# hungkq-1724/EraXviF5TTS

Hardware: AMD Instinct MI355X
Metric: mel-frames/s (higher is better)
Workload: dtype bf16; 1 GPU; C2 F5TTS_Base random-init, CFM.sample euler NFE=32 CFG=2 sway=-1, 32 utterances x seq_len 1024 (N_ref=341), one GPU, hipGraph=on; global_batch=32, per_gpu_batch=32, seq_len=1024, nfe=32, parallelism=utterance-sharded dp1, residual_stream=fp16 storage, fp32 arithmetic

## Files before the change

eraxvif5tts_amd/csrc/gemm_w4.hip:

```cpp
#include "gemm_tile.h"
#include "lnf_stats_math.h"
#include <string.h>

typedef _Float16 f16x4_t __attribute__((ext_vector_type(4)));

namespace {
constexpr int OPB = 32768;
constexpr int EPI_LDS_BYTES = 16384;

template <int EPI, bool LNF, int MI>
__global__ __launch_bounds__(256) __attribute__((amdgpu_waves_per_eu(1, 1))) void gemm_w4_kernel(GemmParams p, int tiles_n, int nblocks) {
    static_assert(EPI == EPI_STORE_T || EPI == EPI_ROPE_T || EPI == EPI_RESID, "block linears only");
    static_assert(!LNF || EPI != EPI_RESID, "LayerNorm fold: QKV (+ RoPE) and FF1 (+ GELU)");
    static_assert(MI == 8 || MI == 4, "token tiles per wave");
    constexpr int WROWS = MI * 16, BM = 2 * WROWS;
    constexpr int OPA = BM * 128;
    constexpr int WBASE = 2 * OPA, EPI_LDS = 2 * OPA + 2 * OPB;
    constexpr int NP = MI + 8, NR = MI + 8, NMF = 16 * MI;
    constexpr int LNF_AREA = MI == 4 ? 11264 : 2048;
    constexpr int EPI_BYTES = 4 * LNF_AREA > EPI_LDS_BYTES ? 4 * LNF_AREA : EPI_LDS_BYTES;
    __shared__ __attribute__((aligned(1024))) char smem[EPI_LDS + EPI_BYTES];
    const int tid = threadIdx.x, lane = tid & 63;
    const int wave = __builtin_amdgcn_readfirstlane(tid >> 6);
    const int wm = wave >> 1, wn = wave & 1;
    const int fr = lane & 15, fq = lane >> 4;

    auto tile_mn = [&](int bid, int& tm0, int& tn0) {
        const int q = nblocks >> 3, r = nblocks & 7, xcd = bid & 7;
        int swz = (xcd < r ? xcd * (q + 1) : r * (q + 1) + (xcd - r) * q) + (bid >> 3);
        if (p.tile_reverse) swz = nblocks - 1 - swz;
        const int gm = p.tile_group > 0 ? p.tile_group : 1;
        const int tiles_m_all = nblocks / tiles_n;
        const int grp = swz / (gm * tiles_n);
        const int gsz = min(gm, tiles_m_all - grp * gm);
        const int rin = swz - grp * gm * tiles_n;
        const int tile_n = rin / gsz, tile_m = grp * gm + (rin - tile_n * gsz);
        tm0 = tile_m * BM;
        tn0 = tile_n * 256;
    };
    [[maybe_unused]] unsigned pfv[4] = {0u, 0u, 0u, 0u};
    if constexpr (MI == 4) {
        if (p.pf_n[0] | p.pf_n[1]) {
#pragma unroll
            for (int r = 0; r < 2; ++r) {
                const size_t line = ((size_t)blockIdx.x * 2 + r) * 256u + tid;
                if (line * 128u < p.pf_n[0]) pfv[r] = *reinterpret_cast<const unsigned*>(static_cast<const char*>(p.pf_p[0]) + line * 128u);
                if (line * 128u < p.pf_n[1]) pfv[2 + r] = *reinterpret_cast<const unsigned*>(static_cast<const char*>(p.pf_p[1]) + line * 128u);
            }
        }
    }
    const int G = gridDim.x;
    const int my_tiles = (nblocks - (int)blockIdx.x + G - 1) / G;
    const int nk = p.K / 64;

    unsigned voffA[MI], voffW[8];
#pragma unroll
    for (int jj = 0; jj < 8; ++jj) {
        const int row = (wave * 8 + jj) * 8 + (lane >> 3);
        const int logical = (lane & 7) ^ ((row >> 1) & 7);
        voffW[jj] = (unsigned)(row * p.ldw * 2 + logical * 16);
    }
#pragma unroll
    for (int jj = 0; jj < MI; ++jj) {
        const int row = (wave * MI + jj) * 8 + (lane >> 3);
        const int logical = (lane & 7) ^ ((row >> 1) & 7);
        voffA[jj] = (unsigned)(row * p.lda * 2 + logical * 16);
    }
    const char* baseA;
    const char* baseW;
    int f_tile = blockIdx.x, f_k = 0;
    auto front_tile = [&]() {
        int sm, sn;
        tile_mn(f_tile, sm, sn);
        baseA = static_cast<const char*>(p.A) + (size_t)sm * p.lda * 2;
        baseW = static_cast<const char*>(p.W) + (size_t)sn * p.ldw * 2;
    };
    front_tile();
    const unsigned lds0 = (unsigned)(size_t)smem;
    const int wdstA = (int)lds0 + wave * MI * 1024, wdstW = (int)lds0 + WBASE + wave * 8192;
    auto dma16w = [&](int ldsdst, unsigned voff, const char* base) {
        asm volatile("s_mov_b32 m0, %0\n\ts_nop 0\n\tglobal_load_lds_dwordx4 %1, %2" ::"s"(ldsdst), "v"(voff), "s"(base) : "memory");
    };
    auto dma4w = [&](int ldsdst, unsigned voff, const void* base) {
        asm volatile("s_mov_b32 m0, %0\n\ts_nop 0\n\tglobal_load_lds_dword %1, %2" ::"s"(ldsdst), "v"(voff), "s"(base) : "memory");
    };
    auto front_advance = [&]() {
        baseA += 128;
        baseW += 128;
        if (++f_k == nk) {
            f_k = 0;
            f_tile += G;
            if (f_tile < nblocks) {
                front_tile();
            } else {
                f_tile -= G;
                baseA -= (size_t)nk * 128;
                baseW -= (size_t)nk * 128;
            }
        }
    };
    const unsigned ra0 = lds0 + (unsigned)((wm * WROWS + fr) * 128 + ((fq ^ (fr >> 1)) * 16));
    const unsigned ra1 = ra0 ^ 64u;
    const unsigned rw0 = lds0 + WBASE + (unsigned)((wn * 128 + fr) * 128 + ((fq ^ (fr >> 1)) * 16));
    const unsigned rw1 = rw0 ^ 64u;

    f32x4 acc[8][MI];
    f32x4 fw[2][8], fa[2][MI];
#define W4_DSR(dst, addr, off) asm volatile("ds_read_b128 %0, %1 offset:%2" : "=v"(dst) : "v"(addr), "n"(off))
    auto rd = [&](auto sc, auto xc, auto ec) {
        constexpr int S = decltype(sc)::value, X = decltype(xc)::value, e = decltype(ec)::value;
        (void)fw; (void)fa; (void)ra0; (void)ra1; (void)rw0; (void)rw1;
        if constexpr (e < 8) {
            if constexpr (S == 0) W4_DSR(fw[0][e], rw0, X * OPB + e * 2048); else W4_DSR(fw[1][e], rw1, X * OPB + e * 2048);
        } else {
            if constexpr (S == 0) W4_DSR(fa[0][e - 8], ra0, X * OPA + (e - 8) * 2048); else W4_DSR(fa[1][e - 8], ra1, X * OPA + (e - 8) * 2048);
        }
    };
    auto body = [&](auto xc, auto waitc) {
        constexpr int X = decltype(xc)::value;
        constexpr bool WAITV = decltype(waitc)::value;
        constexpr int R1S = 1, B1P = MI == 8 ? 20 : 13, D0 = MI == 8 ? 22 : 14, DS = MI == 8 ? 6 : 4, B2P = MI == 8 ? 86 : 42, R0 = MI == 8 ? 88 : 44,
                      R0S = MI == 8 ? 2 : 1;
        static_for<NMF>([&](auto nc) {
            (void)acc; (void)fw; (void)fa; (void)voffA; (void)voffW; (void)baseA; (void)baseW;
            constexpr int n = decltype(nc)::value;
            constexpr int s = n / (8 * MI), i = (n % (8 * MI)) / MI, j = n % MI;
            if constexpr (LNF)
                asm volatile("v_mfma_f32_16x16x32_f16 %0, %1, %2, %0" : "+a"(acc[i][j]) : "v"(fw[s][i]), "v"(fa[s][j]));
            else
                asm volatile("v_mfma_f32_16x16x32_bf16 %0, %1, %2, %0" : "+a"(acc[i][j]) : "v"(fw[s][i]), "v"(fa[s][j]));
            if constexpr (n < NR * R1S && n % R1S == 0) rd(std::integral_constant<int, 1>{}, xc, std::integral_constant<int, n / R1S>{});
            if constexpr (n == B1P) asm volatile("s_waitcnt lgkmcnt(0)\n\ts_barrier" ::: "memory");
            if constexpr (n >= D0 && n < D0 + NP * DS && (n - D0) % DS == 0) {
                constexpr int pc = (n - D0) / DS;
                if constexpr (pc < MI)
                    dma16w(X * OPA + wdstA + pc * 1024, voffA[pc], baseA);
                else
                    dma16w(X * OPB + wdstW + (pc - MI) * 1024, voffW[pc - MI], baseW);
            }
            if constexpr (n == B2P) {
                constexpr int issued = (B2P - D0) / DS + 1 > NP ? NP : (B2P - D0) / DS + 1;
                if constexpr (WAITV)
                    asm volatile("s_waitcnt vmcnt(%0)\n\ts_barrier" ::"n"(issued) : "memory");
                else
                    asm volatile("s_barrier" ::: "memory");
            }
            if constexpr (n >= R0 && n < R0 + NR * R0S && (n - R0) % R0S == 0)
                rd(std::integral_constant<int, 0>{}, std::integral_constant<int, 1 - X>{}, std::integral_constant<int, (n - R0) / R0S>{});
            if constexpr (n == NMF - 1) asm volatile("s_waitcnt lgkmcnt(0)" ::: "memory");
        });
        front_advance();
    };

    using T = std::true_type;
    using F = std::false_type;
    using X0 = std::integral_constant<int, 0>;
    using X1 = std::integral_constant<int, 1>;
    int m0, n0;
    tile_mn(blockIdx.x, m0, n0);
    char* const lnf_lds = smem + EPI_LDS + wave * LNF_AREA;
    [[maybe_unused]] auto stage_lnf = [&]() {
        const int ldst = (int)lds0 + EPI_LDS + wave * LNF_AREA;
        const unsigned nb = (unsigned)(n0 + wn * 128 + lane) * 4u;
        dma4w(ldst, nb, p.lnf_c1);
        dma4w(ldst + 256, nb + 256u, p.lnf_c1);
        dma4w(ldst + 512, nb, p.lnf_c2);
        dma4w(ldst + 768, nb + 256u, p.lnf_c2);
        if constexpr (MI == 4) {
            if (p.lnf_partial) {
                if (lane < 32) {
                    const unsigned ro = (unsigned)((m0 + wm * WROWS + 2 * lane) * 8);
#pragma unroll
                    for (int c = 0; c < 16; ++c)
                        dma16w(ldst + 2048 + c * 512, ro, reinterpret_cast<const char*>(p.lnf_partial + (size_t)c * p.lnf_partial_ld * 2));
                    if (p.lnf_pivot) dma16w(ldst + 2048 + 8192, ro, reinterpret_cast<const char*>(p.lnf_pivot));
                }
                return;
            }
        }
        dma16w(ldst + 1024, (unsigned)((m0 + wm * WROWS + 2 * lane) * 8), reinterpret_cast<const char*>(p.lnf_stats));
    };
    [[maybe_unused]] auto finish_stats = [&]() {
        if constexpr (MI == 4 && LNF) {
            if (p.lnf_partial) {
                float s1 = 0.f, s2 = 0.f;
#pragma unroll
                for (int c = 0; c < 16; ++c) {
                    const f32x2 v = *reinterpret_cast<const f32x2*>(lnf_lds + 2048 + c * 512 + lane * 8);
                    s1 += v[0];
                    s2 += v[1];
                }
                const float pv = p.lnf_pivot ? *reinterpret_cast<const float*>(lnf_lds + 2048 + 8192 + lane * 8) : 0.0f;
                float mean, rstd, sumsq;
                lnf_row_stats(s1, s2, pv, p.K, mean, rstd, sumsq);
                *reinterpret_cast<f32x2*>(lnf_lds + 1024 + lane * 8) = f32x2{mean, rstd};
                if (p.lnf_stats_out && n0 == 0 && wn == 0) {
                    const int m = m0 + wm * WROWS + lane;
                    const bool tok = p.lnf_rows == 0 || m + p.row0 < p.lnf_rows;
                    if (tok) *reinterpret_cast<f32x2*>(p.lnf_stats_out + (size_t)m * 2) = f32x2{mean, rstd};
                    lnf_raise_guard(p.lnf_sat, tok && !(sumsq < 65504.0f * 65504.0f), sumsq, p.lnf_sat_tag, m + p.row0);
                }
            }
        }
    };
    auto load_bias = [&](int tn0, f32x4 (&dst)[8]) {
#pragma unroll
        for (int i = 0; i < 8; ++i) dst[i] = *reinterpret_cast<const f32x4*>(p.bias + tn0 + wn * 128 + i * 16 + 4 * fq);
    };
    auto acc_from = [&](const f32x4 (&b4)[8]) {
        static_for<8>([&](auto ic) {
            static_for<MI>([&](auto jc) { acc[decltype(ic)::value][decltype(jc)::value] = b4[decltype(ic)::value]; });
        });
    };
#define W4_ACC(i, j)                                                                         \
    ([&]() -> f32x4 {                                                                        \
        float c0_, c1_, c2_, c3_;                                                            \
        asm volatile("v_accvgpr_read_b32 %0, %1" : "=v"(c0_) : "a"(acc[i][j][0]));           \
        asm volatile("v_accvgpr_read_b32 %0, %1" : "=v"(c1_) : "a"(acc[i][j][1]));           \
        asm volatile("v_accvgpr_read_b32 %0, %1" : "=v"(c2_) : "a"(acc[i][j][2]));           \
        asm volatile("v_accvgpr_read_b32 %0, %1" : "=v"(c3_) : "a"(acc[i][j][3]));           \
        return f32x4{c0_, c1_, c2_, c3_};                                                    \
    }())

    [[maybe_unused]] auto store_half_impl = [&](auto hc, auto actc, auto ropec) {
        constexpr int h = decltype(hc)::value, ACT = decltype(actc)::value;
        constexpr bool rope_wave = decltype(ropec)::value;
        const int nb = n0 + wn * 128 + h * 64;
        bf16_t* orow = reinterpret_cast<bf16_t*>(p.out_t) + (size_t)(m0 + wm * WROWS + fr) * p.ldo + nb + 16 * (fq & 1) + 8 * (fq >> 1);
        const size_t jstride = (size_t)16 * p.ldo;
        [[maybe_unused]] f32x4 rp[2][4];
        [[maybe_unused]] int pos0 = 0;
        auto load_rope = [&](auto jc, f32x4 (&dst)[4]) {
            constexpr int j = decltype(jc)::value;
            int pos = pos0 + 16 * j;
            pos -= pos >= p.rows_per_batch ? p.rows_per_batch : 0;
            const float* t = p.rope + (size_t)pos * 64 + 4 * fq;
#pragma unroll
            for (int i = 0; i < 4; ++i) dst[i] = *reinterpret_cast<const f32x4*>(t + 16 * i);
        };
        if constexpr (rope_wave) {
            pos0 = (p.row0 + m0 + wm * WROWS + fr) % p.rows_per_batch;
            load_rope(std::integral_constant<int, 0>{}, rp[0]);
        }
        [[maybe_unused]] f32x4 c1h[4], c2h[4];
        [[maybe_unused]] f32x2 stj[2];
        if constexpr (LNF) {
#pragma unroll
            for (int ii = 0; ii < 4; ++ii) {
                c1h[ii] = *reinterpret_cast<const f32x4*>(lnf_lds + ((h * 4 + ii) * 16 + 4 * fq) * 4);
                c2h[ii] = *reinterpret_cast<const f32x4*>(lnf_lds + 512 + ((h * 4 + ii) * 16 + 4 * fq) * 4);
            }
            stj[0] = *reinterpret_cast<const f32x2*>(lnf_lds + 1024 + fr * 8);
        }
        static_for<MI>([&](auto jc) {
            constexpr int j = decltype(jc)::value;
            __builtin_amdgcn_sched_barrier(0);
            if constexpr (LNF && j + 1 < MI) stj[(j + 1) & 1] = *reinterpret_cast<const f32x2*>(lnf_lds + 1024 + ((j + 1) * 16 + fr) * 8);
            if constexpr (rope_wave && j + 1 < MI) load_rope(std::integral_constant<int, j + 1>{}, rp[(j + 1) & 1]);
            f32x4 vals[4];
            static_for<4>([&](auto ic) {
                constexpr int ii = decltype(ic)::value, i = h * 4 + ii;
                f32x4 v = W4_ACC(i, j);
                if constexpr (LNF) v = epi_lnf4(v, stj[j & 1][0], stj[j & 1][1], c1h[ii], c2h[ii]);
                if constexpr (ACT == ACT_GELU_TANH) v = epi_gelu_tanh4(v);
                if constexpr (rope_wave) v = epi_rope4(v, rp[j & 1][ii]);
                vals[ii] = v;
            });
            const u32x4 q0 = pair_swap(to_bf16x4(vals[0]), to_bf16x4(vals[1]));
            const u32x4 q1 = pair_swap(to_bf16x4(vals[2]), to_bf16x4(vals[3]));
            bf16_t* o = orow + j * jstride;
            *reinterpret_cast<u32x4*>(o) = q0;
            *reinterpret_cast<u32x4*>(o + 32) = q1;
        });
    };
    [[maybe_unused]] auto store_half = [&](auto hc, auto actc) {
        if constexpr (EPI == EPI_ROPE_T) {
            const int nb = n0 + wn * 128 + decltype(hc)::value * 64;
            const int part = nb / p.rope_inner;
            if (part < 2 && ((nb - part * p.rope_inner) >> 6) < p.rope_heads) {
                store_half_impl(hc, actc, std::true_type{});
                return;
            }
        }
        store_half_impl(hc, actc, std::false_type{});
    };
    [[maybe_unused]] const float* const lds_bias = reinterpret_cast<const float*>(smem + EPI_LDS);
    [[maybe_unused]] const float* const lds_gate = lds_bias + p.N;
    [[maybe_unused]] auto emit_stats = [&](int nb, int m , float pivot, const f32x4& h0, const f32x4& h1, const f32x4& h2, const f32x4& h3) {
        const f32x4 npv{-pivot, -pivot, -pivot, -pivot};
        const f32x4 d0 = h0 + npv, d1 = h1 + npv, d2 = h2 + npv, d3 = h3 + npv;
        const f32x4 a = (d0 + d1) + (d2 + d3);
        const f32x4 q = __builtin_elementwise_fma(d3, d3, __builtin_elementwise_fma(d2, d2, __builtin_elementwise_fma(d1, d1, d0 * d0)));
        const float s1 = (a[0] + a[1]) + (a[2] + a[3]), s2 = (q[0] + q[1]) + (q[2] + q[3]);
        float a0 = s1, b0 = s2;
        asm volatile("s_nop 1\n\tv_permlane16_swap_b32 %0, %1" : "+v"(a0), "+v"(b0));
        float t = a0 + b0, z = 0.0f;
        asm volatile("s_nop 1\n\tv_permlane32_swap_b32 %0, %1" : "+v"(t), "+v"(z));
        const float tot = t + z;
        if (fq < 2) {
            char* sb = reinterpret_cast<char*>(p.stats_out + ((size_t)(nb >> 6) * p.stats_ld + (m0 + wm * WROWS)) * 2);
            *reinterpret_cast<float*>(sb + (unsigned)((m * 2 + fq) * 4)) = tot;
        }
    };
    [[maybe_unused]] auto resid_tile = [&]() {
        int fr = lane & 15, fq = lane >> 4;
        asm volatile("" : "+v"(fr), "+v"(fq));
        char* const sbase = reinterpret_cast<char*>(p.out_f) + ((size_t)(m0 + wm * WROWS) * p.ldof + n0 + wn * 128) * 2;
        unsigned offj[MI];
#pragma unroll
        for (int j = 0; j < MI; ++j) offj[j] = (unsigned)(((fr + 16 * j) * p.ldof + 16 * (fq & 1) + 8 * (fq >> 1)) * 2);
        unsigned keepbits = 0xffu;
        if (p.rowmask && p.rowbits) keepbits = ((unsigned)p.rowbits[((m0 + wm * WROWS) >> 7) * 16 + fr] >> (((m0 + wm * WROWS) & 127) >> 4)) & ((1u << MI) - 1u);
        float piv[MI];
        if (p.stats_out) {
            const float* pbase = p.stats_pivot ? p.stats_pivot + (size_t)(m0 + wm * WROWS) * 2 : nullptr;
#pragma unroll
            for (int j = 0; j < MI; ++j) piv[j] = pbase ? *reinterpret_cast<const float*>(reinterpret_cast<const char*>(pbase) + (unsigned)((fr + 16 * j) * 8)) : 0.0f;
        }
        u32x4 xs[2][MI][2];
        auto load_step = [&](auto sc) __attribute__((always_inline)) {
            constexpr int h = decltype(sc)::value / MI, j = decltype(sc)::value % MI;
            xs[h][j][0] = *reinterpret_cast<const u32x4*>(sbase + offj[j] + h * 128);
            xs[h][j][1] = *reinterpret_cast<const u32x4*>(sbase + offj[j] + h * 128 + 64);
        };
        constexpr int AHEAD = 4;
        static_for<AHEAD>([&](auto sc) { load_step(sc); });
        __builtin_amdgcn_sched_barrier(0);
        const bool all_kept = __builtin_amdgcn_ballot_w64(keepbits != ((1u << MI) - 1u)) == 0ull;
        auto widen_h = [](unsigned lo, unsigned hi) __attribute__((always_inline)) {
            const f16x4_t hv = __builtin_bit_cast(f16x4_t, u32x2{lo, hi});
            return f32x4{(float)hv[0], (float)hv[1], (float)hv[2], (float)hv[3]};
        };
        auto to_h16 = [](const f32x4& v) __attribute__((always_inline)) {
            f16x4_t hv;
#pragma unroll
            for (int e = 0; e < 4; ++e) hv[e] = (_Float16)__builtin_amdgcn_fmed3f(v[e], -65504.0f, 65504.0f);
            return hv;
        };
        auto h_f32 = [](const f16x4_t& hv) __attribute__((always_inline)) { return f32x4{(float)hv[0], (float)hv[1], (float)hv[2], (float)hv[3]}; };
        auto steps = [&](auto keptc) __attribute__((always_inline)) {
            constexpr bool ALL = decltype(keptc)::value;
            f32x4 g4[4];
            static_for<2 * MI>([&](auto sc) __attribute__((always_inline)) {
                constexpr int h = decltype(sc)::value / MI, j = decltype(sc)::value % MI;
                const int nb = n0 + wn * 128 + h * 64;
                if constexpr (j == 0) {
#pragma unroll
                    for (int ii = 0; ii < 4; ++ii) g4[ii] = *reinterpret_cast<const f32x4*>(lds_gate + nb + ii * 16 + 4 * fq);
                }
                f32x4 x0, x1, x2, x3;
                {
                    const u32x4 q = xs[h][j][0];
                    const u32x2 s0 = __builtin_amdgcn_permlane16_swap(q[0], q[2], false, false);
                    const u32x2 s1 = __builtin_amdgcn_permlane16_swap(q[1], q[3], false, false);
                    x0 = widen_h(s0[0], s1[0]);
                    x1 = widen_h(s0[1], s1[1]);
                }
                {
                    const u32x4 q = xs[h][j][1];
                    const u32x2 s0 = __builtin_amdgcn_permlane16_swap(q[0], q[2], false, false);
                    const u32x2 s1 = __builtin_amdgcn_permlane16_swap(q[1], q[3], false, false);
                    x2 = widen_h(s0[0], s1[0]);
                    x3 = widen_h(s0[1], s1[1]);
                }
                const f32x4 a0 = W4_ACC(h * 4 + 0, j), a1 = W4_ACC(h * 4 + 1, j), a2 = W4_ACC(h * 4 + 2, j), a3 = W4_ACC(h * 4 + 3, j);
                f32x4 v0 = epi_axpy4(a0, g4[0], x0), v1 = epi_axpy4(a1, g4[1], x1), v2 = epi_axpy4(a2, g4[2], x2), v3 = epi_axpy4(a3, g4[3], x3);
                if constexpr (!ALL) {
                    const bool keep = (keepbits >> j) & 1u;
                    v0 = keep ? v0 : x0;
                    v1 = keep ? v1 : x1;
                    v2 = keep ? v2 : x2;
                    v3 = keep ? v3 : x3;
                }
                const f16x4_t h0 = to_h16(v0), h1 = to_h16(v1), h2 = to_h16(v2), h3 = to_h16(v3);
                *reinterpret_cast<u32x4*>(sbase + offj[j] + h * 128) = pair_swap(__builtin_bit_cast(bf16x4, h0), __builtin_bit_cast(bf16x4, h1));
                *reinterpret_cast<u32x4*>(sbase + offj[j] + h * 128 + 64) = pair_swap(__builtin_bit_cast(bf16x4, h2), __builtin_bit_cast(bf16x4, h3));
                if (p.stats_out) emit_stats(nb, fr + 16 * j, piv[j], h_f32(h0), h_f32(h1), h_f32(h2), h_f32(h3));
                if constexpr (decltype(sc)::value + AHEAD < 2 * MI) load_step(std::integral_constant<int, decltype(sc)::value + AHEAD>{});
                __builtin_amdgcn_sched_barrier(0);
            });
        };
        if (all_kept)
            steps(std::true_type{});
        else
            steps(std::false_type{});
    };

    if constexpr (EPI == EPI_RESID) {
        float* lb = reinterpret_cast<float*>(smem + EPI_LDS);
        for (int i = tid; i < p.N; i += 256) {
            lb[i] = p.bias[i];
            lb[p.N + i] = p.gate ? p.gate[i] : 1.0f;
        }
    }
    auto issue_all = [&](int X) {
#pragma unroll
        for (int pc = 0; pc < MI; ++pc) dma16w(X * OPA + wdstA + pc * 1024, voffA[pc], baseA);
#pragma unroll
        for (int pc = 0; pc < 8; ++pc) dma16w(X * OPB + wdstW + pc * 1024, voffW[pc], baseW);
    };
    if constexpr (LNF) stage_lnf();
    issue_all(0);
    front_advance();
    issue_all(1);
    front_advance();
    f32x4 bstart[8];
    if constexpr (LNF) {
#pragma unroll
        for (int i = 0; i < 8; ++i) bstart[i] = f32x4{0.f, 0.f, 0.f, 0.f};
    } else {
        load_bias(n0, bstart);
    }
    acc_from(bstart);
    if constexpr (EPI == EPI_RESID) asm volatile("s_waitcnt lgkmcnt(0)" ::: "memory");
    asm volatile("s_waitcnt vmcnt(%0)\n\ts_barrier" ::"n"(NP) : "memory");
    static_for<NR>([&](auto ec) { rd(std::integral_constant<int, 0>{}, std::integral_constant<int, 0>{}, ec); });
    asm volatile("s_waitcnt lgkmcnt(0)" ::: "memory");

    for (int t = 0; t < my_tiles; ++t) {
        const bool last = t + 1 == my_tiles;
        if (t == 0)
            body(X0{}, T{});
        else
            body(X0{}, F{});
        body(X1{}, T{});
        for (int kt = 2; kt < nk; kt += 2) {
            body(X0{}, T{});
            body(X1{}, T{});
        }
        int nm0 = m0, nn0 = n0;
        if (!last) tile_mn(blockIdx.x + (t + 1) * G, nm0, nn0);
        if constexpr (EPI == EPI_RESID) {
            asm volatile("s_waitcnt vmcnt(0)" ::: "memory");
            __builtin_amdgcn_sched_barrier(0);
            resid_tile();
            __builtin_amdgcn_sched_barrier(0);
            f32x4 bn[8];
#pragma unroll
            for (int i = 0; i < 8; ++i) bn[i] = *reinterpret_cast<const f32x4*>(lds_bias + nn0 + wn * 128 + i * 16 + 4 * fq);
            acc_from(bn);
        } else {
            f32x4 bn[8];
            if constexpr (LNF) {
#pragma unroll
                for (int i = 0; i < 8; ++i) bn[i] = f32x4{0.f, 0.f, 0.f, 0.f};
            } else {
                load_bias(nn0, bn);
#pragma unroll
                for (int i = 0; i < 8; ++i) asm volatile("" ::"v"(bn[i]));
            }
            asm volatile("s_waitcnt vmcnt(0)" ::: "memory");
            __builtin_amdgcn_sched_barrier(0);
            finish_stats();
            if (p.act == ACT_GELU_TANH) {
                store_half(X0{}, std::integral_constant<int, ACT_GELU_TANH>{});
                store_half(X1{}, std::integral_constant<int, ACT_GELU_TANH>{});
            } else {
                store_half(X0{}, std::integral_constant<int, ACT_NONE>{});
                store_half(X1{}, std::integral_constant<int, ACT_NONE>{});
            }
            __builtin_amdgcn_sched_barrier(0);
            acc_from(bn);
        }
        m0 = nm0;
        n0 = nn0;
        if (!last) {
            static_for<NR>([&](auto ec) { rd(std::integral_constant<int, 0>{}, std::integral_constant<int, 0>{}, ec); });
            asm volatile("s_waitcnt lgkmcnt(0)" ::: "memory");
            if constexpr (LNF) stage_lnf();
        }
    }
    if constexpr (MI == 4) {
        if (((pfv[0] ^ pfv[1]) ^ (pfv[2] ^ pfv[3])) == 0x7fc0dead && (p.pf_n[0] | p.pf_n[1]) == 0xffffffffu) p.stats_out[0] = 0.f;
    }
#undef W4_ACC
#undef W4_DSR
}
}

int g_gemm_w4 = 1;
int g_gemm_w4_ink = 1;
int g_gemm_w4_bm = 0;

int gemm_persist_grid();

static int w4_tile_rows(const GemmParams& p) {
    const int pg = gemm_persist_grid();
    const int t256 = p.M % 256 == 0 ? (p.M / 256) * (p.N / 256) : 0, t128 = p.M % 128 == 0 ? (p.M / 128) * (p.N / 256) : 0;
    if (g_gemm_w4_bm == 256) return t256 >= pg ? 256 : 0;
    if (g_gemm_w4_bm == 128) return t128 >= pg ? 128 : 0;
    if (4 * t256 >= 3 * pg) return 256;
    return 2 * t128 >= pg ? 128 : 0;
}

int gemm_w4_lnf_inkernel(int M, int N, int K) {
    GemmParams t;
    memset(&t, 0, sizeof(t));
    t.M = M; t.N = N; t.K = K;
    if (!g_gemm_w4 || !g_gemm_w4_ink || K != 1024 || N % 256 != 0) return 0;
    const int rows = w4_tile_rows(t);
    if (rows == 128) return 128;
    return 0;
}

bool gemm_w4_ok(const GemmParams& p, int mode, int epi) {
    if (!g_gemm_w4 || mode != GEMM_DENSE) return false;
    if (p.N % 256 != 0 || p.K % 128 != 0 || p.K < 256 || (p.lda & 7) || (p.ldw & 7) || p.a_row_mod != 0 || p.row0 != 0) return false;
    if (w4_tile_rows(p) == 0) return false;
    if ((size_t)255 * (size_t)(p.lda > p.ldw ? p.lda : p.ldw) * 2 + 128 > 0x7fffffffull) return false;
    if (p.fin_counter) return false;
    if (p.lnf_partial && !(gemm_w4_lnf_inkernel(p.M, p.N, p.K) != 0 && p.lnf_stats && p.lnf_ncols == 16 && p.lnf_partial_ld >= p.M)) return false;
    const bool lnf = p.lnf_stats != nullptr;
    if (epi == EPI_STORE_T || epi == EPI_ROPE_T) {
        if (!p.out_t || (p.ldo & 7) || !(p.act == ACT_NONE || p.act == ACT_GELU_TANH)) return false;
        if (lnf ? (!p.lnf_c1 || !p.lnf_c2) : !p.bias) return false;
        if (epi == EPI_ROPE_T && (p.rows_per_batch < 128 || !p.rope || p.rope_inner % 64 != 0)) return false;
        return true;
    }
    if (epi == EPI_RESID) {
        if (lnf || !p.add2_f16 || !p.out_f || (p.ldof & 7) || p.act != ACT_NONE || !p.bias) return false;
        if ((p.gate && p.gate_bstride != 0) || (p.rowmask && !p.rowbits)) return false;
        if (p.stats_out && (p.N % 64 != 0 || p.stats_ld < p.M)) return false;
        if ((size_t)p.N * 8 > (size_t)EPI_LDS_BYTES) return false;
        return true;
    }
    return false;
}

template <int MI> static int launch_w4(const GemmParams& p, int epi, hipStream_t stream) {
    const int tiles_n = p.N / 256, nblocks = (p.M / (MI * 32)) * tiles_n;
    const int pg = gemm_persist_grid();
    const dim3 grid(nblocks < pg ? nblocks : pg), block(256);
    const bool lnf = p.lnf_stats != nullptr;
    if (epi == EPI_STORE_T && lnf)
        hipLaunchKernelGGL((gemm_w4_kernel<EPI_STORE_T, true, MI>), grid, block, 0, stream, p, tiles_n, nblocks);
    else if (epi == EPI_STORE_T)
        hipLaunchKernelGGL((gemm_w4_kernel<EPI_STORE_T, false, MI>), grid, block, 0, stream, p, tiles_n, nblocks);
    else if (epi == EPI_ROPE_T && lnf)
        hipLaunchKernelGGL((gemm_w4_kernel<EPI_ROPE_T, true, MI>), grid, block, 0, stream, p, tiles_n, nblocks);
    else if (epi == EPI_ROPE_T)
        hipLaunchKernelGGL((gemm_w4_kernel<EPI_ROPE_T, false, MI>), grid, block, 0, stream, p, tiles_n, nblocks);
    else if (epi == EPI_RESID)
        hipLaunchKernelGGL((gemm_w4_kernel<EPI_RESID, false, MI>), grid, block, 0, stream, p, tiles_n, nblocks);
    else
        return f5_fail(F5_EINVAL, "gemm_w4: unsupported epilogue %d", epi);
    F5_LAUNCH_CHECK();
    return 0;
}

int launch_gemm_w4(const GemmParams& p, int epi, hipStream_t stream) {
    return w4_tile_rows(p) == 128 ? launch_w4<4>(p, epi, stream) : launch_w4<8>(p, epi, stream);
}
```

eraxvif5tts_amd/csrc/ops.hip:

```cpp
#include <cstring>

#include "gemm.h"
#include "kernels.h"
#include "runtime.h"

static int sync_and_release(DevArena& a, hipStream_t st, int rc) {
    hipError_t e = hipStreamSynchronize(st);
    a.release();
    if (rc != 0) return rc;
    if (e != hipSuccess) return f5_fail(F5_EHIP, "stream synchronize failed: %s", hipGetErrorString(e));
    return 0;
}

extern "C" int f5_op_linear(int precision, int kernel, int M, int N, int K, const float* A, const float* W, const float* bias, int act,
                            float* out, f5_stream_t stream) {
    F5_TRY(f5_check_device());
    if (M <= 0 || N <= 0 || K <= 0 || !A || !W || !out) return f5_fail(F5_EINVAL, "bad argument");
    hipStream_t st = (hipStream_t)stream;
    const int Kp = (int)round_up(K, 64), Mp = (int)round_up(M, 256), Np = (int)round_up(N, 256);
    const size_t es = f5_elem_size(precision);
    DevArena a;
    void *At = nullptr, *Wt = nullptr;
    int rc = 0;
    do {
// ... 213 lines not shown
    if (precision != F5_PREC_BF16 && precision != F5_PREC_FP32) return f5_fail(F5_EINVAL, "bad precision %d", precision);
    if (ldx < dim || ldo < dim || (ldx & 3) || (ldo & 3) || (y && (ldy < dim || (ldy & 3)))) return f5_fail(F5_EINVAL, "leading dimensions below dim");
    if ((ymode != 0 && !y) || (ymode == 3 && !y2)) return f5_fail(F5_EINVAL, "residual mode %d needs its branches", ymode);
    if (inplace && xin_f16 != xout_f16) return f5_fail(F5_EINVAL, "in place needs one storage type");
    hipStream_t st = (hipStream_t)stream;
    const size_t es = f5_elem_size(precision), xn = (size_t)rows * ldx;
    DevArena a;
    void *xs = nullptr, *xo = nullptr, *ys = nullptr, *y2s = nullptr, *os = nullptr;
    unsigned* sat = nullptr;
    int rc = 0;
    do {
        if ((rc = a.alloc(&xs, xn * (xin_f16 ? 2 : 4)))) break;
        if ((rc = a.alloc(&os, (size_t)rows * ldo * es))) break;
        if ((rc = a.alloc_t(&sat, 8))) break;
        if (y && (rc = a.alloc(&ys, (size_t)rows * ldy * es))) break;
        if (y2 && (rc = a.alloc(&y2s, (size_t)rows * ldy * es))) break;
        if (inplace) xo = xs;
        else if ((rc = a.alloc(&xo, xn * (xout_f16 ? 2 : 4)))) break;
        if (xin_f16) {
            if ((rc = stage_f16(x, xs, xn, st))) break;
        } else {
            F5_HIP(hipMemcpyAsync(xs, x, xn * 4, hipMemcpyDeviceToDevice, st));
        }
        if (y && (rc = launch_convert_pad(precision, y, ldy, rows, ldy, ldy, ys, ldy, st))) break;
        if (y2 && (rc = launch_convert_pad(precision, y2, ldy, rows, ldy, ldy, y2s, ldy, st))) break;
        if ((rc = launch_layernorm_res(precision, xs, xin_f16, xo, xout_f16, ldx, rows, dim, ys, ldy, y2s, ymode, mul, add, mod_bstride, rows_per_batch,
                                       add_one, os, ldo, st, nullptr, guard ? sat : nullptr, sat_tag)))
            break;
        if ((rc = launch_convert_back(precision, os, ldo, rows, ldo, out, ldo, st))) break;
        if ((rc = xout_f16 ? launch_f16_to_f32(xo, xback, xn, st) : launch_convert_back(F5_PREC_FP32, xo, ldx, rows, ldx, xback, ldx, st))) break;
        if (guard) F5_HIP(hipMemcpyAsync(guard, sat, 6 * sizeof(unsigned), hipMemcpyDeviceToDevice, st));
    } while (0);
    return sync_and_release(a, st, rc);
}

extern "C" int f5_op_f32_to_f16(int64_t n, const float* src, float* dst, uint32_t* guard, f5_stream_t stream) {
    F5_TRY(f5_check_device());
    if (n <= 0 || !src || !dst) return f5_fail(F5_EINVAL, "bad argument");
    hipStream_t st = (hipStream_t)stream;
    DevArena a;
    void* h = nullptr;
    unsigned* sat = nullptr;
    int rc = 0;
    do {
        if ((rc = a.alloc(&h, (size_t)n * 2))) break;
        if ((rc = a.alloc_t(&sat, 8))) break;
        if ((rc = launch_f32_to_f16(src, h, (size_t)n, st, guard ? sat : nullptr))) break;
        if ((rc = launch_f16_to_f32(h, dst, (size_t)n, st))) break;
        if (guard) F5_HIP(hipMemcpyAsync(guard, sat, 6 * sizeof(unsigned), hipMemcpyDeviceToDevice, st));
    } while (0);
    return sync_and_release(a, st, rc);
}

extern "C" int f5_op_qknorm_rope(int precision, int rows, int heads, int rope_heads, int rows_per_batch, const float* qkv, const float* wq,
                                 const float* wk, const float* rope, float* out, f5_stream_t stream) {
    F5_TRY(f5_check_device());
    if (rows <= 0 || heads <= 0 || rope_heads < 0 || rope_heads > heads || rows_per_batch <= 0 || !qkv || !wq || !wk || !out || (rope_heads && !rope))
        return f5_fail(F5_EINVAL, "bad argument");
    if (precision != F5_PREC_BF16 && precision != F5_PREC_FP32) return f5_fail(F5_EINVAL, "bad precision %d", precision);
    hipStream_t st = (hipStream_t)stream;
    const int inner = heads * 64, ld = 3 * inner;
    DevArena a;
    void* q = nullptr;
    int rc = 0;
    do {
        if ((rc = a.alloc(&q, (size_t)rows * ld * f5_elem_size(precision)))) break;
        if ((rc = launch_convert_pad(precision, qkv, ld, rows, ld, ld, q, ld, st))) break;
        if ((rc = launch_qknorm_rope(precision, q, ld, rows, inner, heads, rope_heads, wq, wk, rope, rows_per_batch, st))) break;
        rc = launch_convert_back(precision, q, ld, rows, ld, out, ld, st);
    } while (0);
    return sync_and_release(a, st, rc);
}

extern "C" int f5_op_dwconv7_ln(int precision, int B, int N, int C, const float* x, const float* wt, const float* cbias, const float* ln_w,
                                const float* ln_b, float* out, f5_stream_t stream) {
    F5_TRY(f5_check_device());
    if (B <= 0 || N <= 0 || C <= 0 || !x || !wt || !cbias || !ln_w || !ln_b || !out) return f5_fail(F5_EINVAL, "bad argument");
    if (precision != F5_PREC_BF16 && precision != F5_PREC_FP32) return f5_fail(F5_EINVAL, "bad precision %d", precision);
    hipStream_t st = (hipStream_t)stream;
    const int rows = B * N;
    DevArena a;
    void* o = nullptr;
    int rc = 0;
    do {
        if ((rc = a.alloc(&o, (size_t)rows * C * f5_elem_size(precision)))) break;
        if ((rc = launch_dwconv7_ln(precision, x, B, N, C, wt, cbias, ln_w, ln_b, o, C, st))) break;
        rc = launch_convert_back(precision, o, C, rows, C, out, C, st);
    } while (0);
    return sync_and_release(a, st, rc);
}

extern "C" int f5_op_grn(int precision, int B, int N, int C, const float* h, const float* gamma, const float* beta, float* out, f5_stream_t stream) {
    F5_TRY(f5_check_device());
    if (B <= 0 || N <= 0 || C <= 0 || !h || !gamma || !beta || !out) return f5_fail(F5_EINVAL, "bad argument");
    if (precision != F5_PREC_BF16 && precision != F5_PREC_FP32) return f5_fail(F5_EINVAL, "bad precision %d", precision);
    hipStream_t st = (hipStream_t)stream;
    const int rows = B * N;
    DevArena a;
    void* hs = nullptr;
    float* scratch = nullptr;
    int rc = 0;
    do {
        if ((rc = a.alloc(&hs, (size_t)rows * C * f5_elem_size(precision)))) break;
        if ((rc = a.alloc_t(&scratch, (size_t)B * C + B))) break;
        if ((rc = launch_convert_pad(precision, h, C, rows, C, C, hs, C, st))) break;
        if ((rc = launch_grn(precision, hs, B, N, C, gamma, beta, scratch, st))) break;
        rc = launch_convert_back(precision, hs, C, rows, C, out, C, st);
    } while (0);
    return sync_and_release(a, st, rc);
}

extern "C" int f5_op_rmsnorm(int precision, int rows, int dim, const float* x, const float* g, float* out, f5_stream_t stream) {
    F5_TRY(f5_check_device());
    if (rows <= 0 || dim <= 0 || !x || !g || !out) return f5_fail(F5_EINVAL, "bad argument");
    if (precision != F5_PREC_BF16 && precision != F5_PREC_FP32) return f5_fail(F5_EINVAL, "bad precision %d", precision);
    hipStream_t st = (hipStream_t)stream;
    DevArena a;
    void* o = nullptr;
    int rc = 0;
    do {
        if ((rc = a.alloc(&o, (size_t)rows * dim * f5_elem_size(precision)))) break;
        if ((rc = launch_rmsnorm(precision, x, dim, rows, dim, g, o, dim, st))) break;
        rc = launch_convert_back(precision, o, dim, rows, dim, out, dim, st);
    } while (0);
    return sync_and_release(a, st, rc);
}

__global__ __launch_bounds__(256) void fill_random_kernel(uint16_t* dst, size_t n, uint32_t seed, float scale) {
    const size_t i = (size_t)blockIdx.x * 256 + threadIdx.x;
    if (i >= n) return;
    uint32_t x = (uint32_t)i * 2654435761u ^ seed;
    x ^= x >> 16; x *= 0x7feb352du; x ^= x >> 15; x *= 0x846ca68bu; x ^= x >> 16;
    const float u = ((float)(x >> 8) * (1.0f / 8388608.0f) - 1.0f) * scale;
    dst[i] = (uint16_t)(__float_as_uint(u) >> 16);
}
__global__ __launch_bounds__(256) void fill_random_f32_kernel(float* dst, size_t n, uint32_t seed, float scale) {
    const size_t i = (size_t)blockIdx.x * 256 + threadIdx.x;
    if (i >= n) return;
    uint32_t x = (uint32_t)i * 2654435761u ^ seed;
    x ^= x >> 16; x *= 0x7feb352du; x ^= x >> 15; x *= 0x846ca68bu; x ^= x >> 16;
    dst[i] = ((float)(x >> 8) * (1.0f / 8388608.0f) - 1.0f) * scale;
}

static int g_bench_pad_a = 0, g_bench_pad_w = 0;

extern "C" int f5_bench_gemm_site(int kernel, int site, int rows, int seq, int dim, int heads, int ff_inner, int iters, float* ms_avg,
                                  f5_stream_t stream) {
    F5_TRY(f5_check_device());
    if (!ms_avg || rows <= 0 || iters <= 0 || seq <= 0 || rows % seq != 0) return f5_fail(F5_EINVAL, "bad argument");
    hipStream_t st = (hipStream_t)stream;
    const int inner = heads * 64;
    int N, K, epi;
    switch (site) {
        case 0: N = 3 * inner; K = dim; epi = EPI_ROPE_T; break;
        case 1: N = ff_inner; K = dim; epi = EPI_STORE_T; break;
        case 2: N = dim; K = ff_inner; epi = EPI_GATE_T; break;
        case 3: N = dim; K = inner; epi = EPI_GATE_T; break;
        default: return f5_fail(F5_EINVAL, "bad site");
    }
    const size_t Mp = (size_t)round_up(rows, 256);
    const int lda = K + g_bench_pad_a, ldw = K + g_bench_pad_w;
    DevArena a;
    void *A = nullptr, *W = nullptr, *out = nullptr;
    float *bias = nullptr, *resid = nullptr, *gate = nullptr, *rope = nullptr;
    hipEvent_t e0 = nullptr, e1 = nullptr;
    int rc = 0;
    do {
        if ((rc = a.alloc(&A, Mp * lda * 2))) break;
        if ((rc = a.alloc(&W, (size_t)round_up(N, 256) * ldw * 2))) break;
        if ((rc = a.alloc(&out, Mp * N * 2))) break;
        if ((rc = a.alloc_t(&bias, (size_t)N))) break;
        if ((rc = a.alloc_t(&resid, Mp * (size_t)dim))) break;
        if ((rc = a.alloc_t(&gate, (size_t)dim))) break;
        if ((rc = a.alloc_t(&rope, (size_t)seq * 64))) break;
        hipLaunchKernelGGL(fill_random_kernel, dim3((unsigned)((Mp * lda + 255) / 256)), dim3(256), 0, st, (uint16_t*)A, Mp * lda, 1u, 1.0f);
        hipLaunchKernelGGL(fill_random_kernel, dim3((unsigned)(((size_t)N * ldw + 255) / 256)), dim3(256), 0, st, (uint16_t*)W, (size_t)N * ldw, 2u, 0.05f);
        hipLaunchKernelGGL(fill_random_f32_kernel, dim3((unsigned)((N + 255) / 256)), dim3(256), 0, st, bias, (size_t)N, 3u, 0.1f);
        hipLaunchKernelGGL(fill_random_f32_kernel, dim3((unsigned)((dim + 255) / 256)), dim3(256), 0, st, gate, (size_t)dim, 4u, 0.01f);
        hipLaunchKernelGGL(fill_random_f32_kernel, dim3((unsigned)((seq * 64 + 255) / 256)), dim3(256), 0, st, rope, (size_t)seq * 64, 5u, 0.7f);
        GemmParams g;
        memset(&g, 0, sizeof(g));
        g.A = A; g.lda = lda; g.W = W; g.ldw = ldw; g.M = rows; g.N = N; g.K = K; g.bias = bias; g.rows_per_batch = seq;
        g.site = N == 3 * K ? 1 : (N == K ? 2 : (N == 2 * K ? 3 : (K == 2 * N ? 4 : 0)));
        if (epi == EPI_ROPE_T) { g.out_t = out; g.ldo = N; g.rope = rope; g.rope_inner = inner; g.rope_heads = 1; }
        if (epi == EPI_STORE_T) { g.out_t = out; g.ldo = N; g.act = ACT_GELU_TANH; }
        if (epi == EPI_GATE_T) { g.out_t = out; g.ldo = N; g.gate = gate; g.gate_bstride = 0; }
        if (kernel == 1 && !gemm_fast_supported(g, F5_PREC_BF16, GEMM_DENSE, epi)) { rc = f5_fail(F5_ENOTSUP, "tuned kernel cannot run this site"); break; }
        if (hipEventCreate(&e0) != hipSuccess || hipEventCreate(&e1) != hipSuccess) { rc = f5_fail(F5_EHIP, "hipEventCreate failed"); break; }
        for (int i = 0; i < 2 && rc == 0; ++i) rc = launch_gemm(g, F5_PREC_BF16, GEMM_DENSE, epi, kernel, st);
        if (rc) break;
        (void)hipEventRecord(e0, st);
        for (int i = 0; i < iters && rc == 0; ++i) rc = launch_gemm(g, F5_PREC_BF16, GEMM_DENSE, epi, kernel, st);
        (void)hipEventRecord(e1, st);
        if (rc) break;
        if (hipEventSynchronize(e1) != hipSuccess) { rc = f5_fail(F5_EHIP, "event sync failed: %s", hipGetErrorString(hipGetLastError())); break; }
        float ms = 0.f;
        (void)hipEventElapsedTime(&ms, e0, e1);
        *ms_avg = ms / (float)iters;
    } while (0);
    if (e0) (void)hipEventDestroy(e0);
    if (e1) (void)hipEventDestroy(e1);
    return sync_and_release(a, st, rc);
}

extern "C" int f5_bench_attention(int kernel, int B, int N, int H, int iters, float* ms_avg, f5_stream_t stream) {
    F5_TRY(f5_check_device());
    if (!ms_avg || B <= 0 || N <= 0 || H <= 0 || iters <= 0) return f5_fail(F5_EINVAL, "bad argument");
    hipStream_t st = (hipStream_t)stream;
    const int inner = H * 64;
    const size_t rows = (size_t)B * N;
    DevArena a;
    void *q = nullptr, *o = nullptr;
    hipEvent_t e0 = nullptr, e1 = nullptr;
    int rc = 0;
    do {
        if ((rc = a.alloc(&q, rows * 3 * inner * 2))) break;
        if ((rc = a.alloc(&o, rows * inner * 2))) break;
        hipLaunchKernelGGL(fill_random_kernel, dim3((unsigned)((rows * 3 * inner + 255) / 256)), dim3(256), 0, st, (uint16_t*)q, rows * 3 * inner, 7u, 1.5f);
        if (kernel == 1 && !attention_fast_supported(F5_PREC_BF16, N, H)) { rc = f5_fail(F5_ENOTSUP, "tuned attention cannot run this shape"); break; }
        if (hipEventCreate(&e0) != hipSuccess || hipEventCreate(&e1) != hipSuccess) { rc = f5_fail(F5_EHIP, "hipEventCreate failed"); break; }
        for (int i = 0; i < 2 && rc == 0; ++i) rc = launch_attention(F5_PREC_BF16, kernel, B, N, H, q, 3 * inner, nullptr, o, inner, st);
        if (rc) break;
        (void)hipEventRecord(e0, st);
        for (int i = 0; i < iters && rc == 0; ++i) rc = launch_attention(F5_PREC_BF16, kernel, B, N, H, q, 3 * inner, nullptr, o, inner, st);
        (void)hipEventRecord(e1, st);
        if (rc) break;
        if (hipEventSynchronize(e1) != hipSuccess) { rc = f5_fail(F5_EHIP, "event sync failed"); break; }
        float ms = 0.f;
        (void)hipEventElapsedTime(&ms, e0, e1);
        *ms_avg = ms / (float)iters;
    } while (0);
    if (e0) (void)hipEventDestroy(e0);
    if (e1) (void)hipEventDestroy(e1);
    return sync_and_release(a, st, rc);
}

__global__ __launch_bounds__(256, 1) void mfma_rate_kernel(int iters, int random_operands, float* sink) {
    f32x4 acc[8][8];
#pragma unroll
    for (int i = 0; i < 8; ++i)
#pragma unroll
        for (int j = 0; j < 8; ++j) acc[i][j] = f32x4{0.f, 0.f, 0.f, 0.f};
    bf16x8 w[8], a[8];
    unsigned h = (threadIdx.x * 2654435761u) ^ (blockIdx.x * 40503u);
#pragma unroll
    for (int i = 0; i < 8; ++i)
#pragma unroll
        for (int e = 0; e < 8; ++e) {
            h = h * 1664525u + 1013904223u;
            w[i][e] = random_operands ? (bf16_t)(((int)(h >> 20) & 0xfff) * (1.0f / 1024.0f) - 2.0f) : (bf16_t)0.f;
            h = h * 1664525u + 1013904223u;
            a[i][e] = random_operands ? (bf16_t)(((int)(h >> 20) & 0xfff) * (1.0f / 32768.0f) - 0.0625f) : (bf16_t)0.f;
        }
    for (int it = 0; it < iters; ++it) {
#pragma unroll
        for (int i = 0; i < 8; ++i)
#pragma unroll
            for (int j = 0; j < 8; ++j)
                asm volatile("v_mfma_f32_16x16x32_bf16 %0, %1, %2, %0" : "+a"(acc[i][j]) : "v"(w[i]), "v"(a[j]));
    }
    asm volatile("s_nop 15\n\ts_nop 15" ::: "memory");
    float s = 0.f;
#pragma unroll
    for (int i = 0; i < 8; ++i)
#pragma unroll
        for (int j = 0; j < 8; ++j) s += acc[i][j][0];
    if (s == 12345.678f) sink[0] = s;
}

extern "C" int f5_bench_mfma_rate(int random_operands, float* tflops, f5_stream_t stream) {
    F5_TRY(f5_check_device());
    if (!tflops) return f5_fail(F5_EINVAL, "null argument");
    hipStream_t st = (hipStream_t)stream;
    int dev = 0, cus = 0;
    F5_HIP(hipGetDevice(&dev));
    F5_HIP(hipDeviceGetAttribute(&cus, hipDeviceAttributeMultiprocessorCount, dev));
    const int iters = 2000, blocks = cus * 4;
    DevArena a;
    float* sink = nullptr;
    hipEvent_t e0 = nullptr, e1 = nullptr;
    int rc = 0;
    do {
        if ((rc = a.alloc_t(&sink, 16))) break;
        if (hipEventCreate(&e0) != hipSuccess || hipEventCreate(&e1) != hipSuccess) { rc = f5_fail(F5_EHIP, "hipEventCreate failed"); break; }
        for (int i = 0; i < 3; ++i) hipLaunchKernelGGL(mfma_rate_kernel, dim3(blocks), dim3(256), 0, st, iters, random_operands, sink);
        (void)hipEventRecord(e0, st);
        const int reps = 10;
        for (int i = 0; i < reps; ++i) hipLaunchKernelGGL(mfma_rate_kernel, dim3(blocks), dim3(256), 0, st, iters, random_operands, sink);
        (void)hipEventRecord(e1, st);
        if (hipEventSynchronize(e1) != hipSuccess) { rc = f5_fail(F5_EHIP, "event sync failed"); break; }
        float ms = 0.f;
        (void)hipEventElapsedTime(&ms, e0, e1);
        const double flops = (double)reps * blocks * 4.0 * iters * 64.0 * (2.0 * 16 * 16 * 32);
        *tflops = (float)(flops / (ms * 1e-3) / 1e12);
    } while (0);
    if (e0) (void)hipEventDestroy(e0);
    if (e1) (void)hipEventDestroy(e1);
    return sync_and_release(a, st, rc);
}

extern int g_sync_evals, g_attn_persist, g_attn_stagger, g_resid_rmw, g_ln_fold, g_ln_fold_inkernel, g_ln_fold_fin, g_gemm_pad_rows;
extern int g_conv31_tok;
extern int g_gemm_bm128, g_gemm_tile, g_gemm_group_sites, g_gemm_reverse_sites;
extern int g_gemm_split_tail, g_gemm_w4, g_gemm_w4_bm, g_gemm_w4_ink;
extern int g_gemm_variant, g_gemm_group, g_gemm_persist_grid, g_gemm_persist, g_gemm_lean, g_ln_defer, g_ln_wide, g_ln_rows, g_ln_rows_min, g_w_prefetch, g_res_f16, g_conv31, g_attn_variant, g_vocos_fft;
int g_tuning_epoch = 0;
extern unsigned long long* g_attn_stamp_buf;
extern unsigned long long* g_gemm_clk_buf;
extern "C" int f5_debug_gemm_clock(void* dev_buf) {
    g_gemm_clk_buf = reinterpret_cast<unsigned long long*>(dev_buf);
    return 0;
}
extern "C" int f5_debug_attn_stamps(void* dev_buf) {
    g_attn_stamp_buf = reinterpret_cast<unsigned long long*>(dev_buf);
    return 0;
}

extern "C" int f5_tuning_set(const char* key, int value) {
    if (!key) return f5_fail(F5_EINVAL, "null key");
    ++g_tuning_epoch;
    if (strcmp(key, "gemm_variant") == 0) {
        g_gemm_variant = value;
        return 0;
    }
    if (strcmp(key, "resid_rmw") == 0) {
        g_resid_rmw = value != 0;
        return 0;
    }
    if (strcmp(key, "attn_stagger") == 0) {
        g_attn_stagger = value;
        return 0;
    }
    if (strcmp(key, "attn_persist") == 0) {
        g_attn_persist = value != 0;
        return 0;
    }
    if (strcmp(key, "sync_evals") == 0) {
        g_sync_evals = value != 0;
        return 0;
    }
    if (strcmp(key, "w_prefetch") == 0) {
        g_w_prefetch = value;
        return 0;
    }
    if (strcmp(key, "gemm_reverse_sites") == 0) {
        g_gemm_reverse_sites = value;
        return 0;
    }
    if (strcmp(key, "gemm_group_sites") == 0) {
        g_gemm_group_sites = value;
        return 0;
    }
    if (strcmp(key, "conv31_tok") == 0) {
        g_conv31_tok = value;
        return 0;
    }
    if (strcmp(key, "gemm_tile") == 0) {
        g_gemm_tile = value;
        return 0;
    }
    if (strcmp(key, "gemm_bm128") == 0) {
        g_gemm_bm128 = value;
        return 0;
    }
    if (strcmp(key, "ln_rows") == 0) {
        g_ln_rows = value;
        return 0;
    }
    if (strcmp(key, "ln_rows_min") == 0) {
        g_ln_rows_min = value;
        return 0;
    }
    if (strcmp(key, "ln_wide") == 0) {
        g_ln_wide = value != 0;
        return 0;
    }
    if (strcmp(key, "residual_f16") == 0) {
        g_res_f16 = value != 0;
        return 0;
    }
    if (strcmp(key, "vocos_fft") == 0) {
        g_vocos_fft = value != 0;
        return 0;
    }
    if (strcmp(key, "attn_variant") == 0) {
        g_attn_variant = value;
        return 0;
    }
    if (strcmp(key, "gemm_group") == 0) {
        g_gemm_group = value;
        return 0;
    }
    if (strcmp(key, "op_conv_kernel") == 0) {
        g_op_conv_kernel = value != 0;
        return 0;
    }
    if (strcmp(key, "conv31") == 0) {
        g_conv31 = value != 0;
        return 0;
    }
    if (strcmp(key, "ln_defer") == 0) {
        g_ln_defer = value != 0;
        return 0;
    }
    if (strcmp(key, "gemm_lean") == 0) {
        g_gemm_lean = value != 0;
        return 0;
    }
    if (strcmp(key, "gemm_pad_rows") == 0) {
        g_gemm_pad_rows = value != 0;
        return 0;
    }
    if (strcmp(key, "ln_fold_inkernel") == 0) {
        g_ln_fold_inkernel = value != 0;
        return 0;
    }
    if (strcmp(key, "ln_fold_fin") == 0) {
        g_ln_fold_fin = value != 0;
        return 0;
    }
    if (strcmp(key, "ln_fold") == 0) {
        g_ln_fold = value != 0;
        return 0;
    }
    if (strcmp(key, "gemm_split_tail") == 0) {
        g_gemm_split_tail = value != 0;
        return 0;
    }
    if (strcmp(key, "gemm_w4_ink") == 0) {
        g_gemm_w4_ink = value;
        return 0;
    }
    if (strcmp(key, "gemm_w4_bm") == 0) {
        g_gemm_w4_bm = value;
        return 0;
    }
    if (strcmp(key, "gemm_w4") == 0) {
        g_gemm_w4 = value != 0;
        return 0;
    }
    if (strcmp(key, "gemm_persist") == 0) {
        g_gemm_persist = value != 0;
        return 0;
    }
    if (strcmp(key, "gemm_persist_grid") == 0) {
        if (value != 0 && (value < 8 || value > 4096)) return f5_fail(F5_EINVAL, "gemm_persist_grid must be 0 (= CU count) or in [8, 4096]");
        g_gemm_persist_grid = value;
        return 0;
    }
    if (strcmp(key, "bench_pad_a") == 0) {
        g_bench_pad_a = value;
        return 0;
    }
    if (strcmp(key, "bench_pad_w") == 0) {
        g_bench_pad_w = value;
        return 0;
    }
    return f5_fail(F5_EINVAL, "unknown tuning key '%s'", key);
}
```

Before: 34090 mel-frames/s.

## Defer part of w4 GEMM epilogue stores into next tile's MFMA mainloop

In the persistent w4 GEMM with 256-row tiles, half of the odd token-tile epilogue results (16 u32x4 per wave) are now held in registers. They are written out with global_store_dwordx4 interleaved into the first K-iterations of the next tile, instead of being stored at once in the epilogue. The goal is to overlap epilogue store traffic with MFMA compute. The vmcnt waits are adjusted to count the drained stores, and any leftovers are flushed after the loop. It is enabled by default for RoPE QKV GEMMs only, and it adds register pressure and extra outstanding-store accounting.

```diff
diff --git a/eraxvif5tts_amd/csrc/gemm_w4.hip b/eraxvif5tts_amd/csrc/gemm_w4.hip
--- a/eraxvif5tts_amd/csrc/gemm_w4.hip
+++ b/eraxvif5tts_amd/csrc/gemm_w4.hip
@@ -6,13 +6,16 @@
 
 namespace {
 constexpr int OPB = 32768;
+constexpr int W4_DRAIN = 16;
 constexpr int EPI_LDS_BYTES = 16384;
 
-template <int EPI, bool LNF, int MI>
+template <int EPI, bool LNF, int MI, int ND = 0>
 __global__ __launch_bounds__(256) __attribute__((amdgpu_waves_per_eu(1, 1))) void gemm_w4_kernel(GemmParams p, int tiles_n, int nblocks) {
     static_assert(EPI == EPI_STORE_T || EPI == EPI_ROPE_T || EPI == EPI_RESID, "block linears only");
     static_assert(!LNF || EPI != EPI_RESID, "LayerNorm fold: QKV (+ RoPE) and FF1 (+ GELU)");
     static_assert(MI == 8 || MI == 4, "token tiles per wave");
+    static_assert(ND == 0 || (MI == 8 && EPI != EPI_RESID && ND % 4 == 0 && ND <= 16), "the drain: store-only epilogues of the 256-row tile");
+    constexpr int NJ = ND / 4, NDI = ND / 2;
     constexpr int WROWS = MI * 16, BM = 2 * WROWS;
     constexpr int OPA = BM * 128;
     constexpr int WBASE = 2 * OPA, EPI_LDS = 2 * OPA + 2 * OPB;
@@ -116,9 +119,17 @@
             if constexpr (S == 0) W4_DSR(fa[0][e - 8], ra0, X * OPA + (e - 8) * 2048); else W4_DSR(fa[1][e - 8], ra1, X * OPA + (e - 8) * 2048);
         }
     };
-    auto body = [&](auto xc, auto waitc) {
-        constexpr int X = decltype(xc)::value;
+    u32x4 dq[ND > 0 ? ND : 1];
+    [[maybe_unused]] const char* dbase = static_cast<const char*>(p.out_t);
+    [[maybe_unused]] unsigned doff[NJ > 0 ? NJ : 1];
+    if constexpr (ND > 0) {
+#pragma unroll
+        for (int e = 0; e < ND; ++e) dq[e] = u32x4{0u, 0u, 0u, 0u};
+    }
+    auto body = [&](auto xc, auto waitc, auto stc) {
+        constexpr int X = decltype(xc)::value, ST = decltype(stc)::value;
         constexpr bool WAITV = decltype(waitc)::value;
+        constexpr int DS0 = 97, DS1 = 109;
         constexpr int R1S = 1, B1P = MI == 8 ? 20 : 13, D0 = MI == 8 ? 22 : 14, DS = MI == 8 ? 6 : 4, B2P = MI == 8 ? 86 : 42, R0 = MI == 8 ? 88 : 44,
                       R0S = MI == 8 ? 2 : 1;
         static_for<NMF>([&](auto nc) {
@@ -140,13 +151,19 @@
             }
             if constexpr (n == B2P) {
                 constexpr int issued = (B2P - D0) / DS + 1 > NP ? NP : (B2P - D0) / DS + 1;
+                constexpr int drained = (ND > 0 && ST >= 0) ? (DS0 < B2P ? 1 : 0) + (DS1 < B2P ? 1 : 0) : 0;
                 if constexpr (WAITV)
-                    asm volatile("s_waitcnt vmcnt(%0)\n\ts_barrier" ::"n"(issued) : "memory");
+                    asm volatile("s_waitcnt vmcnt(%0)\n\ts_barrier" ::"n"(issued + drained) : "memory");
                 else
                     asm volatile("s_barrier" ::: "memory");
             }
             if constexpr (n >= R0 && n < R0 + NR * R0S && (n - R0) % R0S == 0)
                 rd(std::integral_constant<int, 0>{}, std::integral_constant<int, 1 - X>{}, std::integral_constant<int, (n - R0) / R0S>{});
+            if constexpr (ND > 0 && ST >= 0 && (n == DS0 || n == DS1)) {
+                constexpr int e = 2 * ST + (n == DS0 ? 0 : 1);
+                (void)dq; (void)doff; (void)dbase;
+                asm volatile("global_store_dwordx4 %0, %1, %2 offset:%3" ::"v"(doff[e / 4]), "v"(dq[e]), "s"(dbase), "n"(64 * (e % 4)) : "memory");
+            }
             if constexpr (n == NMF - 1) asm volatile("s_waitcnt lgkmcnt(0)" ::: "memory");
         });
         front_advance();
@@ -156,6 +173,7 @@
     using F = std::false_type;
     using X0 = std::integral_constant<int, 0>;
     using X1 = std::integral_constant<int, 1>;
+    using N1 = std::integral_constant<int, -1>;
     int m0, n0;
     tile_mn(blockIdx.x, m0, n0);
     char* const lnf_lds = smem + EPI_LDS + wave * LNF_AREA;
@@ -268,9 +286,14 @@
             });
             const u32x4 q0 = pair_swap(to_bf16x4(vals[0]), to_bf16x4(vals[1]));
             const u32x4 q1 = pair_swap(to_bf16x4(vals[2]), to_bf16x4(vals[3]));
-            bf16_t* o = orow + j * jstride;
-            *reinterpret_cast<u32x4*>(o) = q0;
-            *reinterpret_cast<u32x4*>(o + 32) = q1;
+            if constexpr (ND > 0 && (j & 1) && j / 2 < NJ) {
+                dq[(j / 2) * 4 + h * 2] = q0;
+                dq[(j / 2) * 4 + h * 2 + 1] = q1;
+            } else {
+                bf16_t* o = orow + j * jstride;
+                *reinterpret_cast<u32x4*>(o) = q0;
+                *reinterpret_cast<u32x4*>(o + 32) = q1;
+            }
         });
     };
     [[maybe_unused]] auto store_half = [&](auto hc, auto actc) {
@@ -419,14 +442,32 @@
 
     for (int t = 0; t < my_tiles; ++t) {
         const bool last = t + 1 == my_tiles;
-        if (t == 0)
-            body(X0{}, T{});
-        else
-            body(X0{}, F{});
-        body(X1{}, T{});
-        for (int kt = 2; kt < nk; kt += 2) {
-            body(X0{}, T{});
-            body(X1{}, T{});
+        if constexpr (ND == 0) {
+            if (t == 0)
+                body(X0{}, T{}, N1{});
+            else
+                body(X0{}, F{}, N1{});
+            body(X1{}, T{}, N1{});
+            for (int kt = 2; kt < nk; kt += 2) {
+                body(X0{}, T{}, N1{});
+                body(X1{}, T{}, N1{});
+            }
+        } else {
+            int kt = 0;
+            if (t > 0) {
+                static_for<NDI>([&](auto ic) {
+                    constexpr int it = decltype(ic)::value;
+                    if constexpr (it == 0)
+                        body(X0{}, F{}, ic);
+                    else
+                        body(std::integral_constant<int, it & 1>{}, T{}, ic);
+                });
+                kt = NDI;
+            }
+            for (; kt < nk; kt += 2) {
+                body(X0{}, T{}, N1{});
+                body(X1{}, T{}, N1{});
+            }
         }
         int nm0 = m0, nn0 = n0;
         if (!last) tile_mn(blockIdx.x + (t + 1) * G, nm0, nn0);
@@ -459,6 +500,11 @@
                 store_half(X0{}, std::integral_constant<int, ACT_NONE>{});
                 store_half(X1{}, std::integral_constant<int, ACT_NONE>{});
             }
+            if constexpr (ND > 0) {
+                dbase = static_cast<const char*>(p.out_t) + ((size_t)(m0 + wm * WROWS) * p.ldo + n0 + wn * 128) * 2;
+#pragma unroll
+                for (int jd = 0; jd < NJ; ++jd) doff[jd] = (unsigned)(((fr + 16 * (2 * jd + 1)) * p.ldo + 16 * (fq & 1) + 8 * (fq >> 1)) * 2);
+            }
             __builtin_amdgcn_sched_barrier(0);
             acc_from(bn);
         }
@@ -470,6 +516,12 @@
             if constexpr (LNF) stage_lnf();
         }
     }
+    if constexpr (ND > 0) {
+        static_for<ND>([&](auto ec) {
+            constexpr int e = decltype(ec)::value;
+            *reinterpret_cast<u32x4*>(const_cast<char*>(dbase) + doff[e / 4] + 64 * (e % 4)) = dq[e];
+        });
+    }
     if constexpr (MI == 4) {
         if (((pfv[0] ^ pfv[1]) ^ (pfv[2] ^ pfv[3])) == 0x7fc0dead && (p.pf_n[0] | p.pf_n[1]) == 0xffffffffu) p.stats_out[0] = 0.f;
     }
@@ -480,6 +532,7 @@
 
 int g_gemm_w4 = 1;
 int g_gemm_w4_ink = 1;
+int g_gemm_w4_drain = 1;
 int g_gemm_w4_bm = 0;
 
 int gemm_persist_grid();
@@ -532,6 +585,20 @@
     const int pg = gemm_persist_grid();
     const dim3 grid(nblocks < pg ? nblocks : pg), block(256);
     const bool lnf = p.lnf_stats != nullptr;
+    if constexpr (MI == 8) {
+        if ((epi == EPI_ROPE_T ? g_gemm_w4_drain >= 1 : epi == EPI_STORE_T && g_gemm_w4_drain >= 2) && nblocks > (int)grid.x && p.K >= 512 && (size_t)128 * (size_t)p.ldo * 2 < 0x7fffffffull) {
+            if (epi == EPI_STORE_T && lnf)
+                hipLaunchKernelGGL((gemm_w4_kernel<EPI_STORE_T, true, 8, W4_DRAIN>), grid, block, 0, stream, p, tiles_n, nblocks);
+            else if (epi == EPI_STORE_T)
+                hipLaunchKernelGGL((gemm_w4_kernel<EPI_STORE_T, false, 8, W4_DRAIN>), grid, block, 0, stream, p, tiles_n, nblocks);
+            else if (lnf)
+                hipLaunchKernelGGL((gemm_w4_kernel<EPI_ROPE_T, true, 8, W4_DRAIN>), grid, block, 0, stream, p, tiles_n, nblocks);
+            else
+                hipLaunchKernelGGL((gemm_w4_kernel<EPI_ROPE_T, false, 8, W4_DRAIN>), grid, block, 0, stream, p, tiles_n, nblocks);
+            F5_LAUNCH_CHECK();
+            return 0;
+        }
+    }
     if (epi == EPI_STORE_T && lnf)
         hipLaunchKernelGGL((gemm_w4_kernel<EPI_STORE_T, true, MI>), grid, block, 0, stream, p, tiles_n, nblocks);
     else if (epi == EPI_STORE_T)
diff --git a/eraxvif5tts_amd/csrc/ops.hip b/eraxvif5tts_amd/csrc/ops.hip
--- a/eraxvif5tts_amd/csrc/ops.hip
+++ b/eraxvif5tts_amd/csrc/ops.hip
@@ -539,7 +539,7 @@
 extern int g_sync_evals, g_attn_persist, g_attn_stagger, g_resid_rmw, g_ln_fold, g_ln_fold_inkernel, g_ln_fold_fin, g_gemm_pad_rows;
 extern int g_conv31_tok;
 extern int g_gemm_bm128, g_gemm_tile, g_gemm_group_sites, g_gemm_reverse_sites;
-extern int g_gemm_split_tail, g_gemm_w4, g_gemm_w4_bm, g_gemm_w4_ink;
+extern int g_gemm_split_tail, g_gemm_w4, g_gemm_w4_bm, g_gemm_w4_ink, g_gemm_w4_drain;
 extern int g_gemm_variant, g_gemm_group, g_gemm_persist_grid, g_gemm_persist, g_gemm_lean, g_ln_defer, g_ln_wide, g_ln_rows, g_ln_rows_min, g_w_prefetch, g_res_f16, g_conv31, g_attn_variant, g_vocos_fft;
 int g_tuning_epoch = 0;
 extern unsigned long long* g_attn_stamp_buf;
@@ -668,6 +668,10 @@
         g_gemm_w4_ink = value;
         return 0;
     }
+    if (strcmp(key, "gemm_w4_drain") == 0) {
+        g_gemm_w4_drain = value;
+        return 0;
+    }
     if (strcmp(key, "gemm_w4_bm") == 0) {
         g_gemm_w4_bm = value;
         return 0;
```

Result: no change. 34260 mel-frames/s, median of 6 (+0.5%).
